# LuxGraph/Lux

Measured on NVIDIA H100. Metric: MTEPS, higher is better.
Workload: dtype f32

## Files before the change

lux_b200/csrc/api.cu:

```cuda
#include <cub/cub.cuh>
#include <stdarg.h>
#include <stdlib.h>
#include <string.h>
#include <algorithm>
#include <type_traits>
#include <new>

#include "build.cuh"
#include "cf.cuh"
#include "pull.cuh"
#include "panel.cuh"
#include "seg.cuh"
#include "push.cuh"
#include "runtime.cuh"
#include <thrust/iterator/counting_iterator.h>

using namespace luxb;

enum class AppRun : uint8_t { kIterations, kConvergence, kEntry };
static constexpr char kBcRun[] = "luxb_bc_run";

struct AppInfo {
  const char* name;
  AppRun run;
  const char* entry;
  bool weights;
  bool dist_labels;
  uint32_t vbytes;
  bool check;
  bool settable;
};
static constexpr AppInfo kApps[] = {
    {"pagerank",                        AppRun::kIterations,  nullptr,          false,  false, 4,        false, true},
    {"connected components",            AppRun::kConvergence, nullptr,          false,  false, 4,        true,  true},
    {"SSSP",                            AppRun::kConvergence, nullptr,          false,  false, 4,        true,  true},
    {"col_filter",                      AppRun::kIterations,  nullptr,          true,   false, 4 * kCfK, false, true},
    {"weighted SSSP",                   AppRun::kConvergence, nullptr,          true,   true,  4,        true,  true},
    {"betweenness centrality",          AppRun::kEntry,       kBcRun,           false,  false, 8,        false, true},
    {"weighted betweenness centrality", AppRun::kEntry,       kBcRun,           true,   true,  8,        false, true},
    {"triangle counting",               AppRun::kEntry,       "luxb_tc_run",    false,  false, 8,        false, false},
    {"k-core decomposition",            AppRun::kEntry,       "luxb_kcore_run", false,  false, 4,        true,  true},
    {"k-truss decomposition",           AppRun::kEntry,       "luxb_truss_run", false,  false, 4,        true,  false},
};
static constexpr int kNumApps = sizeof(kApps) / sizeof(kApps[0]);
static_assert(kNumApps == LUXB_TRUSS + 1, "one row per luxb_app");
static const AppInfo& app_of(const luxb_graph* g) { return kApps[g->cfg.app]; }

static const char* const kPhaseName[15] = {"pull_tile", "fixup", "refresh", "rechunk", "barrier", "panel", "combine", "pack+push",
                                           "pull/bcast", "cold_hub", "bc_sigma", "bc_delta", "main_join", "join_wait", "overlap"};
static void pt_mark(luxb_graph* g, int tag) {
  PhaseTimer& pt = g->pt;
  if (!pt.on) return;
  cudaEvent_t e;
  cudaEventCreate(&e);
  cudaEventRecord(e, g->stream);
  pt.ev.push_back(e);
  pt.tag.push_back(tag);
}
static int pt_event(luxb_graph* g, cudaStream_t st) {
  PhaseTimer& pt = g->pt;
  if (!pt.on) return -1;
  cudaEvent_t e;
  cudaEventCreate(&e);
  cudaEventRecord(e, st);
  pt.span_ev.push_back(e);
  return (int)pt.span_ev.size() - 1;
}
static void pt_span(luxb_graph* g, int tag, int begin, int end) {
  if (begin >= 0) g->pt.spans.push_back({begin, end, tag});
}
static void pt_print(luxb_graph* g) {
  if (g->pt.on && g->pt.cnt) {
    char line[1024];
    const bool bc = app_of(g).entry == kBcRun;
    int n = snprintf(line, sizeof(line), "[luxb rank %d] phase means over %ld %s:", g->cfg.rank, g->pt.cnt, bc ? "sources" : "iterations");
    double sum = 0;
    for (int k = bc ? 10 : 0; k < (bc ? 12 : 10); ++k) {
      n += snprintf(line + n, sizeof(line) - n, " %s %.3f ms;", kPhaseName[k], g->pt.sum[k] / g->pt.cnt);
      sum += g->pt.sum[k] / g->pt.cnt;
    }
    if (!bc && g->pt.sum[14] > 0) {
      for (int k = 12; k < 15; ++k) n += snprintf(line + n, sizeof(line) - n, " %s %.3f ms;", kPhaseName[k], g->pt.sum[k] / g->pt.cnt);
      sum = g->pt.chain / g->pt.cnt;
    }
    snprintf(line + n, sizeof(line) - n, " sum %.3f ms\n", sum);
    fputs(line, stderr);
  }
}

static void pt_flush(luxb_graph* g) {
  PhaseTimer& pt = g->pt;
  if (!pt.on || pt.ev.empty()) return;
  cudaStreamSynchronize(g->stream);
  const int count_tag = app_of(g).entry == kBcRun ? 10 : 0;
  for (size_t i = 1; i < pt.ev.size(); ++i) {
    if (pt.tag[i] < 0) continue;
    float ms = 0;
    cudaEventElapsedTime(&ms, pt.ev[i - 1], pt.ev[i]);
    pt.sum[pt.tag[i]] += ms;
    pt.chain += ms;
    if (pt.tag[i] == count_tag) pt.cnt++;
  }
  for (const PhaseTimer::Span& s : pt.spans) {
    float ms = 0;
    cudaEventElapsedTime(&ms, pt.span_ev[s.begin], pt.span_ev[s.end]);
    pt.sum[s.tag] += ms;
    if (s.tag == count_tag) pt.cnt++;
  }
  for (cudaEvent_t e : pt.ev) cudaEventDestroy(e);
  for (cudaEvent_t e : pt.span_ev) cudaEventDestroy(e);
  pt.ev.clear();
  pt.tag.clear();
  pt.span_ev.clear();
  pt.spans.clear();
}


namespace luxb {
static thread_local char g_err[1024] = "";
void set_error(const char* fmt, ...) {
  va_list ap;
  va_start(ap, fmt);
  vsnprintf(g_err, sizeof(g_err), fmt, ap);
  va_end(ap);
}
}

#define LUXB_ARG(cond, ...)             \
  do {                                  \
    if (!(cond)) {                      \
      set_error(__VA_ARGS__);           \
      return LUXB_ERR_ARG;              \
    }                                   \
  } while (0)

#define LUXB_NCCL(expr)                                                                              \
  do {                                                                                               \
    ncclResult_t _r = (expr);                                                                        \
    if (_r != ncclSuccess) {                                                                         \
      set_error("NCCL error %s at %s:%d: %s", #expr, __FILE__, __LINE__, nccl().GetErrorString(_r)); \
      return LUXB_ERR_COMM;                                                                          \
    }                                                                                                \
  } while (0)

#define LUXB_PULL_SHAPES(X) X(0, 7, 8, 2) X(1, 9, 8, 2) X(2, 7, 16, 2)
#define LUXB_DECL_SHAPE(id, ipt, warps, stages) using PullShape##id = PullShape<ipt, warps, stages>;
LUXB_PULL_SHAPES(LUXB_DECL_SHAPE)
#define LUXB_TILE_OF(id, ipt, warps, stages) PullShape##id::kTile,
static const int kPullTileOf[] = {LUXB_PULL_SHAPES(LUXB_TILE_OF)};
static const int kNumPullShapes = sizeof(kPullTileOf) / sizeof(int);
static const int kDefaultPullShape = 0;
static const int kDefaultPullCtas = 3;

static inline int grid_for(uint64_t n, int threads, int cap) {
  uint64_t b = (n + threads - 1) / threads;
  if (b < 1) b = 1;
  if (b > (uint64_t)cap) b = cap;
  return (int)b;
}

template <class T>
static size_t padded_bytes(uint64_t count) { return std::max<uint64_t>(count, 1) * sizeof(T) + 256; }
// ... 1522 lines not shown
    cub::DoubleBuffer<uint16_t> kb(d_key, d_key2);
    cub::DoubleBuffer<uint64_t> pb(d_pay, d_pay2);
    int hbits = 1;
    while ((1ull << hbits) < (uint64_t)Nh) ++hbits;
    LUXB_TRY(cub_call(tmp, g->stream, [&](void* t, size_t& b) {
      return cub::DeviceRadixSort::SortPairs(t, b, pb, kb, (long long)g->e_part, 32, 32 + hbits, g->stream);
    }));
    LUXB_TRY(cub_call(tmp, g->stream, [&](void* t, size_t& b) {
      return cub::DeviceRadixSort::SortPairs(t, b, kb, pb, (long long)g->e_part, 0, kSplitKeyBits, g->stream);
    }));
    tmp.release(kb.Alternate());
    tmp.release(pb.Alternate());
    d_key2 = kb.Current();
    d_pay2 = pb.Current();
  }
  uint64_t e_cov = 0, e_cov0 = 0, e_cold = 0;
  for (uint32_t b = 0; b < NB; ++b) e_cov += hist[b];
  for (uint32_t b = 0; b < NB0; ++b) e_cov0 += hist[b];
  for (uint32_t s = 0; s < S; ++s) e_cold += hist[NB + s];
  const uint64_t e_main = hist[kSplitKeyMain];
  if (e_cov + e_cold + e_main != g->e_part) {
    set_error("panel split lost edges (%llu + %llu + %llu != %llu)", (unsigned long long)e_cov, (unsigned long long)e_cold,
              (unsigned long long)e_main, (unsigned long long)g->e_part);
    return LUXB_ERR_STATE;
  }
  if (e_cov == 0 || (st.sb < 0 && e_cov < g->e_part / 5)) return 0;

  const uint32_t NG = NB + S;
  LUXB_ARG(NG < kSplitKeyMain, "panel: too many source groups");
  uint64_t n_pairs = 0, n_words = 0;
  g->sb_groups = SplitGroups{};
  for (uint32_t k = 0; k < NG; ++k) {
    const uint32_t n_k = k < NB ? n_pref[k] : Nh;
    n_pairs += n_k;
    n_words += (n_k + 31) / 32;
    LUXB_ARG(n_pairs < 0x7FFFFFF0ull, "panel: too many (group, hub) pairs");
    g->sb_groups.vbase[k + 1] = (uint32_t)n_pairs;
    g->sb_groups.wbase[k + 1] = (uint32_t)n_words;
  }
  uint32_t *d_slot_bits = nullptr, *d_slot_pre = nullptr;
  LUXB_TRY(tmp.alloc(&d_slot_bits, n_words + 1));
  LUXB_TRY(tmp.alloc(&d_slot_pre, n_words + 1));
  LUXB_TRY(build_group_stream<uint16_t>(g, g->sb_panel, d_key2, d_pay2, e_cov, 0, NB, hist, bs, shp, g->sb_super_end, d_slot_bits, 0));
  if (S)
    LUXB_TRY(build_group_stream<uint32_t>(g, g->sb_cold, d_key2 + e_cov, d_pay2 + e_cov, e_cold, NB, NG, hist, 0,
                                          kSegMainInfo[st.cs_shape], nullptr, d_slot_bits, g->sb_panel.n_slots));
  const uint64_t n_slots = (uint64_t)g->sb_panel.n_slots + (S ? g->sb_cold.n_slots : 0);
  popc_kernel<<<grid, 256, 0, g->stream>>>(d_slot_bits, n_words, d_slot_pre);
  LUXB_CUDA(cudaMemsetAsync(d_slot_pre + n_words, 0, 4, g->stream));
  LUXB_CUDA(cudaGetLastError());
  LUXB_TRY(cub_call(tmp, g->stream, [&](void* t, size_t& b) {
    return cub::DeviceScan::ExclusiveSum(t, b, d_slot_pre, d_slot_pre, (int)n_words + 1, g->stream);
  }));
  uint32_t kind_slots[4] = {0, 0, 0, 0};
  const uint32_t kind_word[4] = {0, g->sb_groups.wbase[NB0], g->sb_groups.wbase[NB], (uint32_t)n_words};
  for (int i = 0; i < 4; ++i) LUXB_CUDA(cudaMemcpyAsync(&kind_slots[i], d_slot_pre + kind_word[i], 4, cudaMemcpyDeviceToHost, g->stream));
  LUXB_CUDA(cudaStreamSynchronize(g->stream));
  if ((uint64_t)kind_slots[3] != n_slots) {
    set_error("panel split: %u slots in the bitmap, %llu in the streams", kind_slots[3], (unsigned long long)n_slots);
    return LUXB_ERR_STATE;
  }

  uint32_t* d_main_src = nullptr;
  uint64_t* d_main_row = nullptr;
  LUXB_TRY(tmp.alloc(&d_main_src, e_main + 8));
  main_fill_kernel<<<grid, 256, 0, g->stream>>>(d_pay2 + e_cov + e_cold, e_main, g->d_src_gather, d_main_src);
  LUXB_TRY(tmp.alloc(&d_main_row, (uint64_t)g->n_part + 4));
  main_indeg_kernel<<<grid, 256, 0, g->stream>>>(g->d_row_end, g->n_part, d_flag, d_hub_idx, d_cov, d_main_row);
  LUXB_CUDA(cudaGetLastError());
  LUXB_TRY(cub_call(tmp, g->stream, [&](void* t, size_t& b) {
    return cub::DeviceScan::InclusiveSum(t, b, d_main_row, d_main_row, (int)g->n_part, g->stream);
  }));
  uint64_t chk = 0;
  LUXB_CUDA(cudaMemcpyAsync(&chk, d_main_row + g->n_part - 1, 8, cudaMemcpyDeviceToHost, g->stream));
  LUXB_CUDA(cudaStreamSynchronize(g->stream));
  if (chk != e_main) { set_error("panel split: offsets do not add up"); return LUXB_ERR_STATE; }
  tmp.release(d_key2);
  tmp.release(d_pay2);
  LUXB_TRY(build_main_stream(g, d_main_row, d_main_src, e_main, d_hub_bits));
  tmp.release(d_main_row);
  tmp.release(d_main_src);

  LUXB_TRY(gmalloc(g, &g->d_sb_partial, (uint64_t)n_slots + 1));
  g->d_hub_vtx = d_hub_vtx; tmp.keep(g, d_hub_vtx);
  g->d_hub_bits = d_hub_bits; tmp.keep(g, d_hub_bits);
  g->d_slot_bits = d_slot_bits; tmp.keep(g, d_slot_bits);
  g->d_slot_pre = d_slot_pre; tmp.keep(g, d_slot_pre);
  g->sb_n_hub = Nh;
  g->sb_n_blocks = NB;
  g->sb_n_groups = NG;
  g->sb_bs = bs;
  g->sb_on = true;
  g->cs_on = S > 0;
  const uint64_t NV = g->sb_groups.vbase[NB];
  g->stats.panel_edges = e_cov0;
  g->stats.panel_hubs = Nh;
  g->stats.panel_blocks = NB0;
  g->stats.cold_hub_edges = e_cold;
  g->stats.cold_hub_segments = S;
  g->stats.tier_blocks = NB - NB0;
  g->stats.tier_slots = NV - (uint64_t)NB0 * Nh;
  g->stats.tier_edges = e_cov - e_cov0;
  if (g->cfg.verbose) {
    printf("[luxb rank %d] source-blocked sweep: %u hub destinations (in-degree >= %u) x %u blocks of %u hot sources, + %u tier blocks "
           "(%llu slots, %llu edges); panel %llu edges (%.1f %%), cold-hub %llu edges (%u segments of %u values), main %llu edges\n",
           g->cfg.rank, Nh, st.sb_min_indeg, NB0, bs, NB - NB0, (unsigned long long)(NV - (uint64_t)NB0 * Nh), (unsigned long long)(e_cov - e_cov0),
           (unsigned long long)e_cov, 100.0 * e_cov / g->e_part, (unsigned long long)e_cold, S, cs.seg, (unsigned long long)e_main);
    printf("[luxb rank %d] (group, hub) pairs with edges / all: tier 0 %u / %llu, tiers %u / %llu, cold segments %u / %llu\n", g->cfg.rank,
           kind_slots[1], (unsigned long long)NB0 * Nh, kind_slots[2] - kind_slots[1], (unsigned long long)(NV - (uint64_t)NB0 * Nh),
           kind_slots[3] - kind_slots[2], (unsigned long long)Nh * S);
  }
  return 0;
}

static int build_seg_sweep(luxb_graph* g) {
  g->seg_on = false;
  g->sb_on = false;
  if (!g->sweep.seg) return 0;
  if (g->n_part == 0 || g->cfg.zero_copy_edges || g->e_part >= 0xFFFFFFF0ull) return 0;
  LUXB_TRY(build_panel_layout(g));
  if (!g->sb_on) LUXB_TRY(build_main_stream(g, g->d_row_end, g->hot_n ? g->d_src_gather : g->d_src, g->e_part, nullptr));
  g->seg_on = true;
  return 0;
}

extern "C++" {
template <class Prog, class Shape>
static int launch_seg_shape(luxb_graph* g, const SegArgs<Prog>& a, int sms, int ctas_per_sm, cudaStream_t st) {
  auto kern = seg_tile_kernel<Prog, Shape>;
  const int reserve = (Shape::kPanel && g->packed) ? g->panel_reserve_sms : 0;
  LUXB_CUDA(cudaFuncSetAttribute(kern, cudaFuncAttributeMaxDynamicSharedMemorySize, (int)Shape::kSmemBytes));
  int carve_pct = (int)std::min<size_t>(100, (ctas_per_sm * (Shape::kSmemBytes + 1024) * 100 + 228 * 1024 - 1) / (228 * 1024));
  LUXB_CUDA(cudaFuncSetAttribute(kern, cudaFuncAttributePreferredSharedMemoryCarveout, carve_pct));
  const uint32_t grid = (uint32_t)std::min<uint64_t>((uint64_t)std::max(std::min(sms, g->num_sms - reserve), 1) * ctas_per_sm, a.n_stages);
  kern<<<grid, Shape::kThreads, Shape::kSmemBytes, st>>>(a);
  LUXB_CUDA(cudaGetLastError());
  return 0;
}

template <class Prog>
static void seg_stream_args(luxb_graph* g, PullLayout& L, SegArgs<Prog>& a, int counter_slot) {
  a.p.tile_v = L.d_tile_v;
  a.p.n_tiles = L.n_tiles;
  fill_fixup_args(a.p, L.fix);
  a.p.close_vtx = L.d_close;
  a.piece_slot = L.d_piece_slot;
  a.words = L.d_src;
  a.n_stages = L.n_stages;
  a.tile_counter = reinterpret_cast<uint32_t*>(g->d_counters + counter_slot);
}

template <bool kPanel, class Prog, bool kSlots = kPanel>
static int launch_seg_kernel(luxb_graph* g, const SegArgs<Prog>& a, int shape, int sms, int ctas_per_sm, cudaStream_t st,
                             const char* name) {
#define LUXB_CASE_MSHAPE(id, warps, stages, rounds) \
  case id: LUXB_TRY((launch_seg_shape<Prog, std::conditional_t<kSlots, SlotShape<SegMain##id>, SegMain##id>>(g, a, sms, ctas_per_sm, st))); break;
#define LUXB_CASE_PSHAPE(id, warps, stages, rounds, tab, v) \
  case id: LUXB_TRY((launch_seg_shape<Prog, SegPanel##id>(g, a, sms, ctas_per_sm, st))); break;
  if constexpr (kPanel) {
    switch (shape) {
      LUXB_SEG_PANEL_SHAPES(LUXB_CASE_PSHAPE)
      default: set_error("bad %s shape", name); return LUXB_ERR_STATE;
    }
  } else {
    switch (shape) {
      LUXB_SEG_MAIN_SHAPES(LUXB_CASE_MSHAPE)
      default: set_error("bad %s shape", name); return LUXB_ERR_STATE;
    }
  }
  g->stats.kernel_launches++;
  return 0;
}

template <bool kPanel, class Prog, bool kSlots = kPanel>
static int launch_seg_stream(luxb_graph* g, PullLayout& L, const SegArgs<Prog>& a, int shape, int ctas_per_sm, int tag, const char* name) {
  LUXB_TRY((launch_seg_kernel<kPanel, Prog, kSlots>(g, a, shape, g->num_sms, ctas_per_sm, g->stream, name)));
  pt_mark(g, tag);
  return launch_fixup(g, a.p, L.fix, L.d_piece_slot);
}
}

extern "C++" {
template <class Prog>
static SegArgs<Prog> seg_main_args(luxb_graph* g, PullLayout& L, const typename Prog::Vertex* x_nat, const typename Prog::Vertex* x_cold,
                                   typename Prog::Vertex* out_local, const typename Prog::Params& prm, const uint32_t* hub_bits) {
  SegArgs<Prog> a{};
  a.p.n_part = L.n_vtx;
  a.p.row_left = g->row_left;
  a.p.x_nat = x_nat;
  a.p.x_old = x_cold;
  a.p.x_hot = reinterpret_cast<const typename Prog::Vertex*>(g->d_hot);
  a.p.hot_n = g->hot_n;
  a.p.out = out_local;
  a.p.prm = prm;
  a.p.hub_bits = hub_bits;
  a.p.l2_hints = g->l2_hints;
  seg_stream_args(g, L, a, 2);
  return a;
}

template <class Prog>
static int launch_seg_empties(luxb_graph* g, PullLayout& L, const PullArgs<Prog>& p, int out_buffer) {
  if (out_buffer >= 0 && L.n_empty && !g->empties_done[out_buffer]) {
    empties_kernel<Prog><<<grid_for(L.n_empty, 256, g->num_sms * 8), 256, 0, g->stream>>>(p, L.d_empty, L.n_empty);
    g->empties_done[out_buffer] = true;
    g->stats.kernel_launches++;
  }
  if (L.n_empty_hub) {
    empties_kernel<Prog><<<grid_for(L.n_empty_hub, 256, g->num_sms * 8), 256, 0, g->stream>>>(p, L.d_empty_hub, L.n_empty_hub);
    g->stats.kernel_launches++;
  }
  LUXB_CUDA(cudaGetLastError());
  return 0;
}

template <class Prog>
static int sweep_seg(luxb_graph* g, const typename Prog::Vertex* x_nat, const typename Prog::Vertex* x_cold, typename Prog::Vertex* out_local,
                     int out_buffer, const typename Prog::Params& prm) {
  using Acc = typename Prog::Acc;
  constexpr bool kColdHub = std::is_same<Prog, PageRankProgram>::value;
  SegArgs<Prog> pa{}, ca{};
  if (g->sb_on) {
    pa.p.x_hot = reinterpret_cast<const typename Prog::Vertex*>(g->d_hot);
    pa.p.out = reinterpret_cast<typename Prog::Vertex*>(g->d_sb_partial);
    pa.p.raw_out = 1;
    pa.p.prm = prm;
    pa.bs = g->sb_bs;
    pa.n_blocks = g->sb_n_blocks;
    for (uint32_t b = 0; b < g->sb_n_blocks; ++b) pa.super_end[b] = g->sb_super_end[b];
    seg_stream_args(g, g->sb_panel, pa, 4);
  }
  if (g->cs_on) {
    if constexpr (kColdHub) {
      ca.p.x_old = x_cold;
      ca.p.x_hot = reinterpret_cast<const typename Prog::Vertex*>(g->d_hot);
      ca.p.hot_n = g->hot_n;
      ca.p.out = reinterpret_cast<typename Prog::Vertex*>(g->d_sb_partial);
      ca.p.raw_out = 1;
      ca.p.l2_hints = 0;
      ca.p.prm = prm;
      seg_stream_args(g, g->sb_cold, ca, 5);
    } else {
      set_error("the cold-hub stream is built for PageRank only");
      return LUXB_ERR_STATE;
    }
  }
  const SegArgs<Prog> ma = seg_main_args<Prog>(g, g->sb_main, x_nat, x_cold, out_local, prm, g->sb_on ? g->d_hub_bits : nullptr);
  const int S = g->sweep.panel_sms;
  const bool beside = g->stream_b && S > 0 && S < g->num_sms;
  LUXB_TRY(kt_begin(g));
  LUXB_CUDA(cudaMemsetAsync(g->d_counters + 2, 0, 4, g->stream));
  if (g->sb_on) LUXB_CUDA(cudaMemsetAsync(g->d_counters + 4, 0, 16, g->stream));
  if (beside) {
    cudaStream_t sb = g->stream_b;
    LUXB_CUDA(cudaEventRecord(g->ev_fork, g->stream));
    const int t_fork = pt_event(g, g->stream);
    LUXB_TRY((launch_seg_kernel<true, Prog>(g, pa, g->sweep.panel_shape, S, 1, g->stream, "panel")));
    pt_mark(g, 5);
    LUXB_CUDA(cudaStreamWaitEvent(sb, g->ev_fork, 0));
    int t = pt_event(g, sb);
    if constexpr (kColdHub) {
      if (g->cs_on) {
        LUXB_TRY((launch_seg_kernel<false, Prog, true>(g, ca, g->sweep.cs_shape, g->num_sms - S, g->pull_ctas, sb, "cold-hub")));
        const int t_cold = pt_event(g, sb);
        pt_span(g, 9, t, t_cold);
        LUXB_TRY(launch_fixup(g, ca.p, g->sb_cold.fix, g->sb_cold.d_piece_slot, sb));
        t = pt_event(g, sb);
        pt_span(g, 1, t_cold, t);
      }
    }
    LUXB_TRY((launch_seg_kernel<false, Prog>(g, ma, g->sweep.main_shape, g->num_sms - S, g->pull_ctas, sb, "seg")));
    pt_span(g, 0, t, pt_event(g, sb));
    LUXB_CUDA(cudaEventRecord(g->ev_join, sb));
    LUXB_TRY(launch_fixup(g, pa.p, g->sb_panel.fix, g->sb_panel.d_piece_slot));
    pt_mark(g, 1);
    LUXB_TRY((launch_seg_kernel<false, Prog>(g, ma, g->sweep.main_shape, S, g->pull_ctas, g->stream, "seg")));
    pt_mark(g, 12);
    LUXB_CUDA(cudaStreamWaitEvent(g->stream, g->ev_join, 0));
    pt_mark(g, 13);
    pt_span(g, 14, t_fork, pt_event(g, g->stream));
  } else {
    if (g->sb_on) {
      LUXB_TRY((launch_seg_stream<true, Prog>(g, g->sb_panel, pa, g->sweep.panel_shape, 1, 5, "panel")));
      pt_mark(g, 1);
    }
    if constexpr (kColdHub) {
      if (g->cs_on) {
        LUXB_TRY((launch_seg_stream<false, Prog, true>(g, g->sb_cold, ca, g->sweep.cs_shape, g->pull_ctas, 9, "cold-hub")));
        pt_mark(g, 1);
      }
    }
    LUXB_TRY(wait_cold_exchange(g));
    LUXB_TRY((launch_seg_kernel<false, Prog>(g, ma, g->sweep.main_shape, g->num_sms, g->pull_ctas, g->stream, "seg")));
    pt_mark(g, 0);
  }
  LUXB_TRY(launch_fixup(g, ma.p, g->sb_main.fix, g->sb_main.d_piece_slot));
  LUXB_TRY(launch_seg_empties(g, g->sb_main, ma.p, out_buffer));
  pt_mark(g, 1);
  LUXB_TRY(kt_end(g));
  if (g->sb_on) {
    CombineArgs<Prog> cb{};
    cb.hub_vtx = g->d_hub_vtx;
    cb.n_hub = g->sb_n_hub;
    cb.n_blocks = g->sb_n_blocks;
    cb.n_groups = g->sb_n_groups;
    cb.row_left = g->row_left;
    cb.sg = g->sb_groups;
    cb.slot_bits = g->d_slot_bits;
    cb.slot_pre = g->d_slot_pre;
    cb.partial = reinterpret_cast<const Acc*>(g->d_sb_partial);
    cb.x_nat = x_nat;
    cb.out = out_local;
    cb.prm = prm;
    combine_hub_kernel<Prog><<<grid_for(g->sb_n_hub, 256, g->num_sms * 8), 256, 0, g->stream>>>(cb);
    LUXB_CUDA(cudaGetLastError());
    g->stats.kernel_launches++;
    pt_mark(g, 6);
  }
  return 0;
}
}

static int pagerank_publish(luxb_graph* g, float* x_new) {
  const int me = g->cfg.rank;
  const int grid = g->num_sms * 8;
  if (g->P == 1 || !g->packed) {
    if (g->P > 1) { LUXB_TRY(allgather_slices(g, x_new, 4)); pt_mark(g, 3); }
    if (g->hot_n) {
      const uint32_t z_n = g->hot_n + (g->cold_z ? g->cold_n : 0);
      hot_refresh_kernel<float><<<grid_for(z_n, 256, grid), 256, 0, g->stream>>>((float*)g->d_hot, x_new, g->d_hot_order, 0, z_n);
      LUXB_CUDA(cudaGetLastError());
      g->stats.kernel_launches++;
      pt_mark(g, 2);
    }
    return 0;
  }
  LUXB_TRY(wait_cold_exchange(g));
  float* XTn = g->d_xt[1 - g->cur_xt];
  const uint32_t H = g->hot_n;
  const uint64_t Ch = g->xt_hot_chunk, Cc = g->xt_cold_chunk, cold_base = Ch * g->P;
  const uint32_t nh_me = g->hot_off[me + 1] - g->hot_off[me], nc_me = g->cold_off[me + 1] - g->cold_off[me];
  const bool p2p = g->p2p_ready && g->cfg.exchange != LUXB_EXCHANGE_NCCL;
  if (p2p) {
    if (nh_me + nc_me) {
      PackPushArgs<float> pa{};
      pa.x_local = x_new + g->row_left;
      pa.list = g->d_pack_list;
      pa.n_hot = nh_me;
      pa.n_cold = nc_me;
      pa.hot_pos0 = g->hot_off[me];
      pa.cold_pos0 = g->cold_off[me];
      pa.hot_chunk = Ch;
      pa.cold_chunk = Cc;
      pa.cold_base = cold_base;
      for (int k = 0; k < g->P; ++k) pa.xt[k] = reinterpret_cast<float*>(g->peer_xt[1 - g->cur_xt][k]);
      pa.P = g->P;
      const int pgrid = grid_for((uint64_t)nh_me + nc_me, 256, grid);
      if (g->direct_push) pack_push_kernel<float, true><<<pgrid, 256, 0, g->stream>>>(pa);
      else pack_push_kernel<float, false><<<pgrid, 256, 0, g->stream>>>(pa);
      LUXB_CUDA(cudaGetLastError());
      g->stats.kernel_launches++;
    }
    pt_mark(g, 7);
    LUXB_TRY(p2p_barrier(g));
    pt_mark(g, 4);
    auto pull = [&](uint64_t base, uint64_t C, cudaStream_t st, int ctas) -> int {
      ChunkPullArgs ca{};
      ca.dst = XTn + base;
      for (int k = 0; k < g->P; ++k) ca.src[k] = reinterpret_cast<const float*>(g->peer_xt[1 - g->cur_xt][k]) + base;
      ca.chunk = C;
      ca.P = g->P;
      ca.me = me;
      chunk_pull_kernel<<<ctas, 512, 0, st>>>(ca);
      LUXB_CUDA(cudaGetLastError());
      g->stats.kernel_launches++;
      return 0;
    };
    if (g->direct_push) {
    } else if (g->overlap_exchange) {
      LUXB_CUDA(cudaEventRecord(g->ev_pack, g->stream));
      LUXB_TRY(pull(0, Ch, g->stream, g->num_sms * 2));
      LUXB_CUDA(cudaStreamWaitEvent(g->stream2, g->ev_pack, 0));
      LUXB_TRY(pull(cold_base, Cc, g->stream2, std::max(2 * g->panel_reserve_sms, 8)));
      LUXB_CUDA(cudaEventRecord(g->ev_cold, g->stream2));
      g->cold_pending = true;
    } else {
      LUXB_TRY(pull(0, Ch, g->stream, g->num_sms * 2));
      LUXB_TRY(pull(cold_base, Cc, g->stream, g->num_sms * 2));
    }
    pt_mark(g, 8);
  } else {
    if (nh_me + nc_me) {
      pack_values_kernel<float><<<grid_for((uint64_t)nh_me + nc_me, 256, grid), 256, 0, g->stream>>>(
// ... 1527 lines not shown
```

lux_b200/csrc/panel.cuh:

```cuda
#pragma once
#include "common.cuh"
#include "programs.cuh"
#include "pull.cuh"

namespace luxb {

constexpr int kPanelMaxBlocks = 256;
constexpr uint16_t kSplitKeyMain = 511;
constexpr int kSplitKeyBits = 9;

struct SplitGroups {
  uint32_t vbase[kSplitKeyMain + 1];
  uint32_t wbase[kSplitKeyMain + 1];
};

__global__ void hub_flag_kernel(const uint64_t* __restrict__ row_end_rel, uint32_t n_part, uint32_t min_indeg,
                                uint32_t* __restrict__ flag) {
  for (uint64_t i = (uint64_t)blockIdx.x * blockDim.x + threadIdx.x; i < n_part; i += (uint64_t)gridDim.x * blockDim.x) {
    uint64_t d = row_end_rel[i] - (i == 0 ? 0 : row_end_rel[i - 1]);
    flag[i] = d >= min_indeg ? 1u : 0u;
  }
}

__global__ void hub_list_kernel(const uint32_t* __restrict__ flag, const uint32_t* __restrict__ hub_idx, uint32_t n_part,
// ... 50 lines not shown
    for (uint64_t k = b + lane; k < e; k += 32) {
      const uint32_t id = src_gather[k];
      if (id < n_src) {
        if (h < s_pref[id / bs]) {
          key[k] = (uint16_t)(id / bs);
          payload[k] = (h << 32) | k;
          ++cnt;
        }
      } else if (cs.seg != 0 && id >= cs.hot_n) {
        key[k] = (uint16_t)(cs.key0 + (id - cs.hot_n) / cs.seg);
        payload[k] = (h << 32) | k;
        ++cnt;
      }
    }
#pragma unroll
    for (int off = 16; off; off >>= 1) cnt += __shfl_xor_sync(0xffffffffu, cnt, off);
    if (lane == 0) cov_count[h] = cnt;
  }
}

__global__ void key_hist_kernel(const uint16_t* __restrict__ key, uint64_t n, unsigned long long* __restrict__ hist) {
  constexpr int kBins = kSplitKeyMain + 1;
  __shared__ unsigned int s_h[kBins];
  for (int i = threadIdx.x; i < kBins; i += blockDim.x) s_h[i] = 0;
  __syncthreads();
  for (uint64_t e = (uint64_t)blockIdx.x * blockDim.x + threadIdx.x; e < n; e += (uint64_t)gridDim.x * blockDim.x)
    atomicAdd(&s_h[key[e]], 1u);
  __syncthreads();
  for (int i = threadIdx.x; i < kBins; i += blockDim.x)
    if (s_h[i]) atomicAdd(hist + i, (unsigned long long)s_h[i]);
}

template <class Word>
__global__ void group_fill_kernel(const uint16_t* __restrict__ key_sorted, const uint64_t* __restrict__ payload_sorted, uint64_t e_cnt,
                                  const uint32_t* __restrict__ src_gather, uint32_t bs, const __grid_constant__ SplitGroups sg,
                                  uint32_t v0, Word* __restrict__ ids, uint32_t* __restrict__ vcount) {
  for (uint64_t i = (uint64_t)blockIdx.x * blockDim.x + threadIdx.x; i < e_cnt; i += (uint64_t)gridDim.x * blockDim.x) {
    const uint32_t k = key_sorted[i];
    const uint64_t p = payload_sorted[i];
    const uint32_t e = (uint32_t)p, h = (uint32_t)(p >> 32);
    ids[i] = (Word)(src_gather[e] - k * bs);
    atomicAdd(vcount + (sg.vbase[k] - v0) + h, 1u);
  }
}

__global__ void main_fill_kernel(const uint64_t* __restrict__ payload_sorted, uint64_t e_main, const uint32_t* __restrict__ src_gather,
                                 uint32_t* __restrict__ main_src) {
  for (uint64_t i = (uint64_t)blockIdx.x * blockDim.x + threadIdx.x; i < e_main; i += (uint64_t)gridDim.x * blockDim.x)
    main_src[i] = src_gather[(uint32_t)payload_sorted[i]];
}

__global__ void main_indeg_kernel(const uint64_t* __restrict__ row_end_rel, uint32_t n_part, const uint32_t* __restrict__ flag,
                                  const uint32_t* __restrict__ hub_idx, const uint32_t* __restrict__ cov_count,
                                  uint64_t* __restrict__ out) {
  for (uint64_t i = (uint64_t)blockIdx.x * blockDim.x + threadIdx.x; i < n_part; i += (uint64_t)gridDim.x * blockDim.x) {
    uint64_t d = row_end_rel[i] - (i == 0 ? 0 : row_end_rel[i - 1]);
    if (flag[i]) d -= cov_count[hub_idx[i]];
    out[i] = d;
  }
}

__global__ void slot_bits_kernel(const uint32_t* __restrict__ vcount, const __grid_constant__ SplitGroups sg, uint32_t g0, uint32_t g1,
                                 uint32_t v0, uint32_t* __restrict__ bits) {
  const unsigned lane = threadIdx.x & 31;
  const uint64_t warps_total = ((uint64_t)gridDim.x * blockDim.x) >> 5;
  for (uint64_t w = sg.wbase[g0] + (((uint64_t)blockIdx.x * blockDim.x + threadIdx.x) >> 5); w < sg.wbase[g1]; w += warps_total) {
    uint32_t lo = g0, hi = g1;
    while (hi - lo > 1) {
      const uint32_t mid = (lo + hi) >> 1;
      if (sg.wbase[mid] <= w) lo = mid; else hi = mid;
    }
    const uint32_t h = (uint32_t)(w - sg.wbase[lo]) * 32u + lane;
    const bool f = h < sg.vbase[lo + 1] - sg.vbase[lo] && vcount[sg.vbase[lo] - v0 + h] != 0;
    const unsigned m = __ballot_sync(0xffffffffu, f);
    if (lane == 0) bits[w] = m;
  }
}

__global__ void popc_kernel(const uint32_t* __restrict__ bits, uint64_t n, uint32_t* __restrict__ out) {
  for (uint64_t i = (uint64_t)blockIdx.x * blockDim.x + threadIdx.x; i < n; i += (uint64_t)gridDim.x * blockDim.x) out[i] = __popc(bits[i]);
}

template <class Prog>
struct CombineArgs {
  const uint32_t* hub_vtx;
  uint32_t n_hub, n_blocks, n_groups, row_left;
  SplitGroups sg;
  const uint32_t* slot_bits;
  const uint32_t* slot_pre;
  const typename Prog::Acc* partial;
  const typename Prog::Vertex* x_nat;
  typename Prog::Vertex* out;
  typename Prog::Params prm;
};

template <class Prog>
__global__ void combine_hub_kernel(const __grid_constant__ CombineArgs<Prog> a) {
  for (uint64_t h = (uint64_t)blockIdx.x * blockDim.x + threadIdx.x; h < a.n_hub; h += (uint64_t)gridDim.x * blockDim.x) {
    const uint32_t v = a.hub_vtx[h];
    typename Prog::Acc raw0;
    memcpy(&raw0, &a.out[v], sizeof(raw0));
    typename Prog::Wide t = Prog::widen(raw0);
    const uint32_t w = (uint32_t)(h >> 5), me = 1u << (h & 31), below = me - 1u;
    auto add8 = [&](uint32_t g) {
      uint32_t bits[8], pre[8];
#pragma unroll
      for (int i = 0; i < 8; ++i) {
        bits[i] = __ldg(a.slot_bits + a.sg.wbase[g + i] + w);
        pre[i] = __ldg(a.slot_pre + a.sg.wbase[g + i] + w);
      }
      typename Prog::Acc p[8];
#pragma unroll
      for (int i = 0; i < 8; ++i) p[i] = (bits[i] & me) ? a.partial[pre[i] + __popc(bits[i] & below)] : Prog::identity();
#pragma unroll
      for (int i = 0; i < 8; ++i)
        if (bits[i] & me) t = Prog::wcombine(t, Prog::widen(p[i]));
    };
    auto add = [&](uint32_t g) {
      const uint32_t bits = __ldg(a.slot_bits + a.sg.wbase[g] + w);
      if (bits & me) t = Prog::wcombine(t, Prog::widen(a.partial[__ldg(a.slot_pre + a.sg.wbase[g] + w) + __popc(bits & below)]));
    };
    uint32_t b = 0;
    for (; b + 8 <= a.n_blocks && h < a.sg.vbase[b + 8] - a.sg.vbase[b + 7]; b += 8) add8(b);
    for (; b < a.n_blocks && h < a.sg.vbase[b + 1] - a.sg.vbase[b]; ++b) add(b);
    uint32_t k = a.n_blocks;
    for (; k + 8 <= a.n_groups; k += 8) add8(k);
    for (; k < a.n_groups; ++k) add(k);
    const typename Prog::Vertex oldv = Prog::kNeedsOld ? a.x_nat[a.row_left + v] : typename Prog::Vertex();
    const typename Prog::Vertex nv_ = Prog::update(a.row_left + v, Prog::narrow(t), oldv, a.prm);
    a.out[v] = nv_;
  }
}

}
```

lux_b200/csrc/runtime.cuh:

```cuda
#pragma once
#include <vector>
#include "comm.h"
#include "common.cuh"
#include "panel.cuh"
#include "seg.cuh"
#include "push.cuh"
#include "bc.cuh"
#include "tc.cuh"
#include "kcore.cuh"
#include "truss.cuh"

struct FixupScratch {
  void* d_head = nullptr;
  void* d_tail = nullptr;
  void* d_carry = nullptr;
  uint32_t* d_carry_flag = nullptr;
  void* d_block_agg = nullptr;
  uint32_t* d_block_flag = nullptr;
  uint32_t n_fix_blocks = 0;
  unsigned long long* d_chain = nullptr;
  uint32_t chain_epoch = 0;
};

struct PullLayout {
  uint64_t* d_row_end = nullptr;
  uint32_t* d_row_end32 = nullptr;
  void* d_src = nullptr;
  uint32_t* d_tile_v = nullptr;
  uint32_t n_vtx = 0;
  uint64_t e_cnt = 0;
  uint32_t n_tiles = 0;
  FixupScratch fix;
  uint32_t* d_close = nullptr;
  uint2* d_piece_slot = nullptr;
  uint32_t n_slots = 0;
  uint32_t* d_empty = nullptr;
  uint32_t n_empty = 0;
  uint32_t* d_empty_hub = nullptr;
  uint32_t n_empty_hub = 0;
  uint32_t n_stages = 0;
  uint64_t n_words = 0;
};

struct SweepSettings {
  bool seg = true;
  int main_shape = 6, panel_shape = 1, cs_shape = 6;
  int sb = -1;
  uint32_t sb_bs = 0;
  uint32_t sb_blocks = 48;
  uint32_t sb_min_indeg = 64;
  int sb_tier = -1;
  double sb_slot_edges = 0.5;
  int cs = -1;
  double cs_seg_mb = 24.0;
  double hot_mb = 24.0;
  bool l2_persist = true;
  double l2_window_mb = -1.0;
  int panel_sms = 40;
};

struct PhaseTimer {
  struct Span { int begin, end, tag; };
  bool on = false, per_call = false;
  std::vector<cudaEvent_t> ev;
  std::vector<int> tag;
  std::vector<cudaEvent_t> span_ev;
  std::vector<Span> spans;
  double sum[15] = {0};
  double chain = 0;
  long cnt = 0;
};

struct CfState {
  uint32_t* chunk_first = nullptr;
  uint32_t* chunk_vtx = nullptr;
  uint32_t n_chunks = 0;
  float* partial = nullptr;
};

struct BcState {
  double* sigma = nullptr;
  double* delta = nullptr;
  double* scores = nullptr;
  uint32_t* order = nullptr;
  double* lvl = nullptr;
  uint64_t lvl_cap = 0;
  uint32_t* off = nullptr;
  uint64_t off_cap = 0;
  uint32_t* split = nullptr;
  uint64_t split_cap = 0;
  void* sort_tmp = nullptr;
  size_t sort_bytes = 0;
  uint32_t* ctl = nullptr;
  luxb::BcHub* hubs = nullptr;
  double* partial = nullptr;
  std::vector<uint32_t> h_off, h_split;
  bool has_source = false;
};

struct TcState {
  uint64_t m = 0;
  uint64_t* off = nullptr;
  uint32_t* dst = nullptr;
  uint32_t* staged = nullptr;
  uint64_t* stage_pre = nullptr;
  uint32_t* group = nullptr;
  uint32_t* big = nullptr;
  uint32_t n_group = 0, n_big = 0;
  unsigned long long* t = nullptr;
  unsigned long long* total = nullptr;
  unsigned int* next = nullptr;
  void* sum_tmp = nullptr;
  size_t sum_bytes = 0;
  int group_grid = 0, big_grid = 0;
};

struct KcoreState {
  uint64_t m = 0;
  uint64_t* off = nullptr;
  uint32_t* adj = nullptr;
  uint32_t* deg0 = nullptr;
  uint32_t* deg = nullptr;
  uint32_t* core = nullptr;
  uint32_t* alive[2] = {nullptr, nullptr};
  uint32_t* piece[2] = {nullptr, nullptr};
  uint32_t* f = nullptr;
  uint64_t* pre = nullptr;
  luxb::KcoreRec* rec = nullptr;
  luxb::KcoreRec* h_rec = nullptr;
  unsigned long long* bad = nullptr;
  void* scan_tmp = nullptr;
  size_t scan_bytes = 0;
  int grid = 0;
};

struct TrussState {
  uint64_t m = 0;
  uint32_t e_lo = 0, e_hi = 0;
  uint64_t* ekey = nullptr;
  TcState o;
  uint32_t* oid = nullptr;
  uint64_t* off = nullptr;
  uint64_t* adj = nullptr;
  uint32_t* sup0 = nullptr;
  uint32_t* sup = nullptr;
  uint32_t* truss = nullptr;
  uint8_t* st = nullptr;
  uint32_t* tv = nullptr;
  uint32_t* alive[2] = {nullptr, nullptr};
  uint32_t* piece[2] = {nullptr, nullptr};
  uint32_t* f = nullptr;
// ... 31 lines not shown

  uint32_t row_left = 0, n_part = 0;
  uint64_t col_left = 0, e_part = 0;
  uint64_t* d_row_end = nullptr;
  uint32_t* d_src = nullptr;
  int32_t* d_weight = nullptr;
  PullLayout base;
  int pull_shape = 0;

  cudaStream_t stream = nullptr;
  cudaEvent_t ev_begin = nullptr, ev_end = nullptr;
  int num_sms = 0;

  bool inited = false;
  uint32_t* d_deg = nullptr;
  void* d_val[2] = {nullptr, nullptr};
  int cur = 0;
  uint32_t hot_n = 0;
  void* d_hot = nullptr;
  uint32_t hot_off[LUXB_MAX_PARTS + 1]{};
  uint32_t* d_hot_order = nullptr;
  uint32_t* d_src_gather = nullptr;
  bool packed = false;
  uint32_t cold_n = 0;
  uint32_t cold_off[LUXB_MAX_PARTS + 1]{};
  uint32_t* d_zperm = nullptr;
  uint32_t* d_pack_list = nullptr;
  float* d_xt[2] = {nullptr, nullptr};
  int cur_xt = 0;
  uint64_t xt_hot_chunk = 0, xt_cold_chunk = 0;
  cudaStream_t stream2 = nullptr;
  cudaEvent_t ev_pack = nullptr, ev_cold = nullptr;
  bool cold_pending = false;

  void* peer_xt[2][LUXB_MAX_PARTS]{};
  bool replica_stale = false;
  uint32_t* d_cur = nullptr;
  uint64_t* d_out_end = nullptr;
  uint32_t* d_out_dst = nullptr;
  int32_t* d_out_w = nullptr;
  void* d_big_list = nullptr;
  uint32_t big_capacity = 0;
  unsigned char* d_fq_all = nullptr;
  unsigned char* d_fq_new = nullptr;
  unsigned char* d_fq_tmp = nullptr;
  uint32_t* d_hdr_all = nullptr;
  luxb::FrontierCtl* d_fctl = nullptr;
  uint64_t* d_slot_off = nullptr;
  uint32_t* h_hdr = nullptr;
  uint32_t* h_scratch = nullptr;
  unsigned long long* d_counters = nullptr;
  CfState cf;
  BcState bc;
  TcState tc;
  KcoreState kc;
  TrussState tr;

  luxb::ncclComm_t comm = nullptr;
  bool p2p_ready = false;
  void* peer_val[2][LUXB_MAX_PARTS]{};
  void* peer_fq[LUXB_MAX_PARTS]{};
  uint32_t* d_sync = nullptr;
  uint32_t* d_flags = nullptr;
  void* peer_flags[LUXB_MAX_PARTS]{};
  uint32_t barrier_epoch = 0;
  uint32_t* h_barrier_err = nullptr;
  uint64_t barrier_timeout_ns = 30000000000ull;
  bool flag_barrier = true;
  bool flag_barrier_all = false;
  bool direct_push = false;

  SweepSettings sweep;

  bool empties_done[2] = {false, false};
  bool seg_on = false;
  bool sb_on = false;
  PullLayout sb_main, sb_panel;
  uint32_t sb_n_hub = 0, sb_n_blocks = 0, sb_n_groups = 0, sb_bs = 0;
  uint32_t* d_hub_vtx = nullptr;
  uint32_t* d_hub_bits = nullptr;
  uint32_t* d_sb_partial = nullptr;
  uint32_t* d_slot_bits = nullptr;
  uint32_t* d_slot_pre = nullptr;
  luxb::SplitGroups sb_groups{};
  uint32_t sb_super_end[luxb::kPanelMaxBlocks]{};
  bool cold_z = false;
  bool cs_on = false;
  PullLayout sb_cold;
  cudaStream_t stream_b = nullptr;
  cudaEvent_t ev_fork = nullptr, ev_join = nullptr;

  int pull_ctas = 3;
  bool overlap_exchange = true;
  bool fused_fixup = true;
  int panel_reserve_sms = 12;
  int l2_hints = 1;
  PhaseTimer pt;

  bool kernel_timing = false;
  std::vector<cudaEvent_t> kt_events;
  size_t kt_used = 0;

  std::vector<OwnedBuf> owned;

  luxb_stats_t stats{};
  std::vector<uint64_t> trace_active;
  std::vector<int32_t> trace_pull;
};
```

Baseline: 211,700.

## Precompute panel hub sums in a warp-cooperative kernel before combine

New measurement: 213,000 (median of 6 runs). Within noise of the previous version (+0.6%).

```diff
diff --git a/lux_b200/csrc/api.cu b/lux_b200/csrc/api.cu
--- a/lux_b200/csrc/api.cu
+++ b/lux_b200/csrc/api.cu
@@ -46,8 +46,9 @@
 static_assert(kNumApps == LUXB_TRUSS + 1, "one row per luxb_app");
 static const AppInfo& app_of(const luxb_graph* g) { return kApps[g->cfg.app]; }
 
-static const char* const kPhaseName[15] = {"pull_tile", "fixup", "refresh", "rechunk", "barrier", "panel", "combine", "pack+push",
-                                           "pull/bcast", "cold_hub", "bc_sigma", "bc_delta", "main_join", "join_wait", "overlap"};
+static const char* const kPhaseName[16] = {"pull_tile", "fixup", "refresh", "rechunk", "barrier", "panel", "combine", "pack+push",
+                                           "pull/bcast", "cold_hub", "bc_sigma", "bc_delta", "main_join", "join_wait", "overlap",
+                                           "panel_sum"};
 static void pt_mark(luxb_graph* g, int tag) {
   PhaseTimer& pt = g->pt;
   if (!pt.on) return;
@@ -78,6 +79,10 @@
     for (int k = bc ? 10 : 0; k < (bc ? 12 : 10); ++k) {
       n += snprintf(line + n, sizeof(line) - n, " %s %.3f ms;", kPhaseName[k], g->pt.sum[k] / g->pt.cnt);
       sum += g->pt.sum[k] / g->pt.cnt;
+    }
+    if (!bc && g->pt.sum[15] > 0) {
+      n += snprintf(line + n, sizeof(line) - n, " %s %.3f ms;", kPhaseName[15], g->pt.sum[15] / g->pt.cnt);
+      sum += g->pt.sum[15] / g->pt.cnt;
     }
     if (!bc && g->pt.sum[14] > 0) {
       for (int k = 12; k < 15; ++k) n += snprintf(line + n, sizeof(line) - n, " %s %.3f ms;", kPhaseName[k], g->pt.sum[k] / g->pt.cnt);
@@ -1766,6 +1771,7 @@
   tmp.release(d_main_src);
 
   LUXB_TRY(gmalloc(g, &g->d_sb_partial, (uint64_t)n_slots + 1));
+  LUXB_TRY(gmalloc(g, &g->d_panel_sum, (uint64_t)Nh + 1));
   g->d_hub_vtx = d_hub_vtx; tmp.keep(g, d_hub_vtx);
   g->d_hub_bits = d_hub_bits; tmp.keep(g, d_hub_bits);
   g->d_slot_bits = d_slot_bits; tmp.keep(g, d_slot_bits);
@@ -1899,9 +1905,29 @@
 }
 
 template <class Prog>
+static SlotTable<Prog> slot_table(luxb_graph* g) {
+  SlotTable<Prog> t{};
+  t.sg = g->sb_groups;
+  t.slot_bits = g->d_slot_bits;
+  t.slot_pre = g->d_slot_pre;
+  t.partial = reinterpret_cast<const typename Prog::Acc*>(g->d_sb_partial);
+  return t;
+}
+
+template <class Prog>
+static int launch_panel_sum(luxb_graph* g, int sms) {
+  const uint32_t grid = (uint32_t)std::min<uint64_t>((uint64_t)sms * 8, ((uint64_t)g->sb_n_hub + 255) / 256);
+  panel_sum_kernel<Prog><<<std::max(grid, 1u), 256, 0, g->stream>>>(slot_table<Prog>(g), g->sb_n_hub, g->sb_n_blocks,
+                                                                    reinterpret_cast<typename Prog::Wide*>(g->d_panel_sum));
+  LUXB_CUDA(cudaGetLastError());
+  g->stats.kernel_launches++;
+  pt_mark(g, 15);
+  return 0;
+}
+
+template <class Prog>
 static int sweep_seg(luxb_graph* g, const typename Prog::Vertex* x_nat, const typename Prog::Vertex* x_cold, typename Prog::Vertex* out_local,
                      int out_buffer, const typename Prog::Params& prm) {
-  using Acc = typename Prog::Acc;
   constexpr bool kColdHub = std::is_same<Prog, PageRankProgram>::value;
   SegArgs<Prog> pa{}, ca{};
   if (g->sb_on) {
@@ -1958,6 +1984,7 @@
     LUXB_CUDA(cudaEventRecord(g->ev_join, sb));
     LUXB_TRY(launch_fixup(g, pa.p, g->sb_panel.fix, g->sb_panel.d_piece_slot));
     pt_mark(g, 1);
+    LUXB_TRY(launch_panel_sum<Prog>(g, S));
     LUXB_TRY((launch_seg_kernel<false, Prog>(g, ma, g->sweep.main_shape, S, g->pull_ctas, g->stream, "seg")));
     pt_mark(g, 12);
     LUXB_CUDA(cudaStreamWaitEvent(g->stream, g->ev_join, 0));
@@ -1967,6 +1994,7 @@
     if (g->sb_on) {
       LUXB_TRY((launch_seg_stream<true, Prog>(g, g->sb_panel, pa, g->sweep.panel_shape, 1, 5, "panel")));
       pt_mark(g, 1);
+      LUXB_TRY(launch_panel_sum<Prog>(g, g->num_sms));
     }
     if constexpr (kColdHub) {
       if (g->cs_on) {
@@ -1989,10 +2017,8 @@
     cb.n_blocks = g->sb_n_blocks;
     cb.n_groups = g->sb_n_groups;
     cb.row_left = g->row_left;
-    cb.sg = g->sb_groups;
-    cb.slot_bits = g->d_slot_bits;
-    cb.slot_pre = g->d_slot_pre;
-    cb.partial = reinterpret_cast<const Acc*>(g->d_sb_partial);
+    cb.st = slot_table<Prog>(g);
+    cb.panel_sum = reinterpret_cast<const typename Prog::Wide*>(g->d_panel_sum);
     cb.x_nat = x_nat;
     cb.out = out_local;
     cb.prm = prm;
diff --git a/lux_b200/csrc/panel.cuh b/lux_b200/csrc/panel.cuh
--- a/lux_b200/csrc/panel.cuh
+++ b/lux_b200/csrc/panel.cuh
@@ -156,13 +156,73 @@
 }
 
 template <class Prog>
-struct CombineArgs {
-  const uint32_t* hub_vtx;
-  uint32_t n_hub, n_blocks, n_groups, row_left;
+struct SlotTable {
   SplitGroups sg;
   const uint32_t* slot_bits;
   const uint32_t* slot_pre;
   const typename Prog::Acc* partial;
+};
+
+template <class Prog, int K>
+__device__ __forceinline__ void add_groups(typename Prog::Wide& t, const SlotTable<Prog>& s, uint32_t g, uint32_t w, uint32_t me) {
+  uint32_t bits[K], idx[K];
+#pragma unroll
+  for (int i = 0; i < K; ++i) {
+    bits[i] = __ldg(s.slot_bits + s.sg.wbase[g + i] + w);
+    idx[i] = __ldg(s.slot_pre + s.sg.wbase[g + i] + w) + __popc(bits[i] & (me - 1u));
+  }
+  typename Prog::Acc p[K];
+#pragma unroll
+  for (int i = 0; i < K; ++i) p[i] = s.partial[idx[i]];
+#pragma unroll
+  for (int i = 0; i < K; ++i)
+    if (bits[i] & me) t = Prog::wcombine(t, Prog::widen(p[i]));
+}
+
+constexpr int kPanelSumGroups = 32;
+
+template <class Prog>
+__global__ void __launch_bounds__(256) panel_sum_kernel(const __grid_constant__ SlotTable<Prog> s, uint32_t n_hub, uint32_t n_blocks,
+                                                        typename Prog::Wide* __restrict__ sum) {
+  constexpr uint32_t K = kPanelSumGroups;
+  const unsigned lane = threadIdx.x & 31;
+  const uint32_t n_words = (n_hub + 31) >> 5, warps = (gridDim.x * blockDim.x) >> 5;
+  for (uint32_t w = (blockIdx.x * blockDim.x + threadIdx.x) >> 5; w < n_words; w += warps) {
+    uint32_t lo = 0, hi = n_blocks;
+    while (lo < hi) {
+      const uint32_t mid = (lo + hi) >> 1;
+      if (w * 32u < s.sg.vbase[mid + 1] - s.sg.vbase[mid]) lo = mid + 1; else hi = mid;
+    }
+    typename Prog::Wide t = Prog::widen(Prog::identity());
+    for (uint32_t b = 0; b < lo; b += K) {
+      uint32_t my_bits = 0, my_pre = 0;
+      if (b + lane < lo) {
+        my_bits = __ldg(s.slot_bits + s.sg.wbase[b + lane] + w);
+        my_pre = __ldg(s.slot_pre + s.sg.wbase[b + lane] + w);
+      }
+      uint32_t hit = 0;
+      typename Prog::Acc p[K];
+#pragma unroll
+      for (uint32_t i = 0; i < K; ++i) {
+        const uint32_t bits = __shfl_sync(0xffffffffu, my_bits, i), pre = __shfl_sync(0xffffffffu, my_pre, i);
+        hit |= ((bits >> lane) & 1u) << i;
+        p[i] = s.partial[pre + __popc(bits & ((1u << lane) - 1u))];
+      }
+#pragma unroll
+      for (uint32_t i = 0; i < K; ++i)
+        if (hit & (1u << i)) t = Prog::wcombine(t, Prog::widen(p[i]));
+    }
+    const uint32_t h = w * 32u + lane;
+    if (h < n_hub) sum[h] = t;
+  }
+}
+
+template <class Prog>
+struct CombineArgs {
+  const uint32_t* hub_vtx;
+  uint32_t n_hub, n_blocks, n_groups, row_left;
+  SlotTable<Prog> st;
+  const typename Prog::Wide* panel_sum;
   const typename Prog::Vertex* x_nat;
   typename Prog::Vertex* out;
   typename Prog::Params prm;
@@ -174,32 +234,11 @@
     const uint32_t v = a.hub_vtx[h];
     typename Prog::Acc raw0;
     memcpy(&raw0, &a.out[v], sizeof(raw0));
-    typename Prog::Wide t = Prog::widen(raw0);
-    const uint32_t w = (uint32_t)(h >> 5), me = 1u << (h & 31), below = me - 1u;
-    auto add8 = [&](uint32_t g) {
-      uint32_t bits[8], pre[8];
-#pragma unroll
-      for (int i = 0; i < 8; ++i) {
-        bits[i] = __ldg(a.slot_bits + a.sg.wbase[g + i] + w);
-        pre[i] = __ldg(a.slot_pre + a.sg.wbase[g + i] + w);
-      }
-      typename Prog::Acc p[8];
-#pragma unroll
-      for (int i = 0; i < 8; ++i) p[i] = (bits[i] & me) ? a.partial[pre[i] + __popc(bits[i] & below)] : Prog::identity();
-#pragma unroll
-      for (int i = 0; i < 8; ++i)
-        if (bits[i] & me) t = Prog::wcombine(t, Prog::widen(p[i]));
-    };
-    auto add = [&](uint32_t g) {
-      const uint32_t bits = __ldg(a.slot_bits + a.sg.wbase[g] + w);
-      if (bits & me) t = Prog::wcombine(t, Prog::widen(a.partial[__ldg(a.slot_pre + a.sg.wbase[g] + w) + __popc(bits & below)]));
-    };
-    uint32_t b = 0;
-    for (; b + 8 <= a.n_blocks && h < a.sg.vbase[b + 8] - a.sg.vbase[b + 7]; b += 8) add8(b);
-    for (; b < a.n_blocks && h < a.sg.vbase[b + 1] - a.sg.vbase[b]; ++b) add(b);
+    typename Prog::Wide t = Prog::wcombine(a.panel_sum[h], Prog::widen(raw0));
+    const uint32_t w = (uint32_t)(h >> 5), me = 1u << (h & 31);
     uint32_t k = a.n_blocks;
-    for (; k + 8 <= a.n_groups; k += 8) add8(k);
-    for (; k < a.n_groups; ++k) add(k);
+    for (; k + 8 <= a.n_groups; k += 8) add_groups<Prog, 8>(t, a.st, k, w, me);
+    for (; k < a.n_groups; ++k) add_groups<Prog, 1>(t, a.st, k, w, me);
     const typename Prog::Vertex oldv = Prog::kNeedsOld ? a.x_nat[a.row_left + v] : typename Prog::Vertex();
     const typename Prog::Vertex nv_ = Prog::update(a.row_left + v, Prog::narrow(t), oldv, a.prm);
     a.out[v] = nv_;
diff --git a/lux_b200/csrc/runtime.cuh b/lux_b200/csrc/runtime.cuh
--- a/lux_b200/csrc/runtime.cuh
+++ b/lux_b200/csrc/runtime.cuh
@@ -56,7 +56,7 @@
   double hot_mb = 24.0;
   bool l2_persist = true;
   double l2_window_mb = -1.0;
-  int panel_sms = 40;
+  int panel_sms = 48;
 };
 
 struct PhaseTimer {
@@ -66,7 +66,7 @@
   std::vector<int> tag;
   std::vector<cudaEvent_t> span_ev;
   std::vector<Span> spans;
-  double sum[15] = {0};
+  double sum[16] = {0};
   double chain = 0;
   long cnt = 0;
 };
@@ -264,6 +264,7 @@
   uint32_t* d_sb_partial = nullptr;
   uint32_t* d_slot_bits = nullptr;
   uint32_t* d_slot_pre = nullptr;
+  uint64_t* d_panel_sum = nullptr;
   luxb::SplitGroups sb_groups{};
   uint32_t sb_super_end[luxb::kPanelMaxBlocks]{};
   bool cold_z = false;
```
